# Sun-Sir/BSARec

Measured on AMD Instinct MI355X. Metric: train sequences/sec, ML-1M L=50 d=64 2-layer, higher is better.
Workload: dtype f32

## Files before the change

### bsarec_amd/csrc/fused_layer.h

```cpp
#pragma once
#include "common.h"
#include "kernels.h"
#include "wimage.h"
#include <type_traits>

#define FS 68
#define FU 260
#define FUSED_MAX_CB 8

struct FusedFwdP {
    const float* X; float* Xout;
    const float *sqrt_beta, *f_g, *f_b, *wq, *bq, *wk, *bk, *wv, *bv, *wo, *bo, *a_g, *a_b, *w1, *b1, *w2, *b2, *ff_g, *ff_b;
    const float* tw; const int* ids32;
    float *xhat_f, *rstd_f, *q, *k, *v, *probs, *ctx, *xhat_a, *rstd_a, *hmix, *u, *xhat_ff, *rstd_ff, *dsp;
    float* gp;
    int L, Lp, cb, heads;
    float alpha, oma, eps;
    DropP drop_f, drop_p, drop_o, drop_ff;
    float* trash;
    long long* stamps;
    const float *e_E, *e_pos, *e_g, *e_b; const int64_t* e_ids; GatherP e_gp; DropP e_drop; int e_V;
    float *e_X0, *e_xhat, *e_rstd; int* e_ids32;
    int xout_f32;
    const float* filter_cw;
// ... 175 lines not shown
#pragma unroll
        for (int s = 0; s < K / 16; ++s) { f.w[2 * s] = gld4(base + e + 16 * s); f.w[2 * s + 1] = gld4(base + e + 16 * s + 4); }
    } else {
#pragma unroll
        for (int kb = 0; kb < K / 8; ++kb) f.w[kb] = gld4(base + e + 8 * kb);
    }
}
template <int MM, int K, int LDW, int NR = 64, bool IMG = false>
__device__ __forceinline__ void load_wT(const float* __restrict__ base, long e, WFrag<MM, K>& f) {
    static_assert(!IMG || MM == 0, "the fragment image exists for the fp32 products only");
    if constexpr (IMG) {
        const float* gw = base + wimage_off((int)(e % LDW), (int)(e / LDW), NR);
#pragma unroll
        for (int kb = 0; kb < K / 8; ++kb) f.w[kb] = gld4(gw + 256 * kb);
    } else if constexpr (MM == 1) {
        const AS_GLOBAL unsigned short* g = reinterpret_cast<const AS_GLOBAL unsigned short*>((const AS_GLOBAL char*)base + 2 * e);
#pragma unroll
        for (int s = 0; s < K / 16; ++s) {
            unsigned h[8];
#pragma unroll
            for (int j = 0; j < 8; ++j) h[j] = g[(16 * s + j) * LDW];
            f.w[s] = u32x4{h[0] | (h[1] << 16), h[2] | (h[3] << 16), h[4] | (h[5] << 16), h[6] | (h[7] << 16)};
        }
    } else if constexpr (MM == 2) {
        const float* gw = base + e;
#pragma unroll
        for (int s = 0; s < K / 16; ++s) {
            f.w[2 * s] = f32x4{gld(gw + (16 * s + 0) * LDW), gld(gw + (16 * s + 1) * LDW), gld(gw + (16 * s + 2) * LDW), gld(gw + (16 * s + 3) * LDW)};
            f.w[2 * s + 1] = f32x4{gld(gw + (16 * s + 4) * LDW), gld(gw + (16 * s + 5) * LDW), gld(gw + (16 * s + 6) * LDW), gld(gw + (16 * s + 7) * LDW)};
        }
    } else {
        const float* gw = base + e;
#pragma unroll
        for (int kb = 0; kb < K / 8; ++kb) {
            f.w[kb].x = gld(gw + (8 * kb + 0) * LDW); f.w[kb].y = gld(gw + (8 * kb + 1) * LDW);
            f.w[kb].z = gld(gw + (8 * kb + 2) * LDW); f.w[kb].w = gld(gw + (8 * kb + 3) * LDW);
        }
    }
}
template <int MM, int K>
__device__ __forceinline__ void mma_w(const float* __restrict__ sa, const WFrag<MM, K>& f, f32x16& acc) {
    if constexpr (MM == 1) {
#pragma unroll
        for (int s = 0; s < K / 16; ++s) acc = mfma_bf16(pk8(ld4(sa + 16 * s), ld4(sa + 16 * s + 4)), f.w[s], acc);
    } else if constexpr (MM == 2) {
#pragma unroll
        for (int s = 0; s < K / 16; ++s)
            acc = mfma_x3(split3(ld4(sa + 16 * s), ld4(sa + 16 * s + 4)), split3(f.w[2 * s], f.w[2 * s + 1]), acc);
    } else {
#pragma unroll
        for (int kb = 0; kb < K / 8; ++kb) {
            const f32x4 a = ld4(sa + 8 * kb);
#pragma unroll
            for (int s = 0; s < 4; ++s) acc = __builtin_amdgcn_mfma_f32_32x32x2f32(a[s], f.w[kb][s], acc, 0, 0, 0);
        }
    }
}
template <int MM, int K>
__device__ __forceinline__ void mma_ll(const float* __restrict__ sa, const float* __restrict__ sb, f32x16& acc) {
    if constexpr (MM == 1) {
#pragma unroll
        for (int s = 0; s < K / 16; ++s)
            acc = mfma_bf16(pk8(ld4(sa + 16 * s), ld4(sa + 16 * s + 4)), pk8(ld4(sb + 16 * s), ld4(sb + 16 * s + 4)), acc);
    } else if constexpr (MM == 2) {
#pragma unroll
        for (int s = 0; s < K / 16; ++s)
            acc = mfma_x3(split3(ld4(sa + 16 * s), ld4(sa + 16 * s + 4)), split3(ld4(sb + 16 * s), ld4(sb + 16 * s + 4)), acc);
    } else {
#pragma unroll
        for (int kb = 0; kb < K / 8; ++kb) {
            const f32x4 a = ld4(sa + 8 * kb), b = ld4(sb + 8 * kb);
#pragma unroll
            for (int s = 0; s < 4; ++s) acc = __builtin_amdgcn_mfma_f32_32x32x2f32(a[s], b[s], acc, 0, 0, 0);
        }
    }
}

struct LnPre { f32x4 bi, g, be, dm[2]; };
__device__ __forceinline__ LnPre ln_pre(const float* __restrict__ bias, const float* __restrict__ gamma, const float* __restrict__ beta,
                                        const DropP& drop, const DropSeed& dseed, long tok0) {
    const int lr = threadIdx.x >> 4, lc = (threadIdx.x & 15) << 2;
    LnPre P;
    P.bi = gld4(bias + lc); P.g = gld4(gamma + lc); P.be = gld4(beta + lc);
#pragma unroll
    for (int i = 0; i < 2; ++i) P.dm[i] = drop_mult4(drop, dseed, (uint64_t)((tok0 + lr + 32 * i) * 64 + lc) >> 2);
    return P;
}
template <bool MIX, bool BF>
__device__ __forceinline__ void ln_rows_64(const LnPre& P, const float* __restrict__ tileA, const float* __restrict__ tileB,
                                           const float* __restrict__ resid, float eps, const float* __restrict__ dsp,
                                           float alpha, float oma, long tok0, int L, float* __restrict__ outL,
                                           float* __restrict__ outG, float* __restrict__ xhatG, float* __restrict__ rstdG,
                                           bool out_f32 = false ,
                                           bool round_outL = false ) {
    const int lr = threadIdx.x >> 4, lc = (threadIdx.x & 15) << 2;
#pragma unroll
    for (int i = 0; i < 2; ++i) {
        const int r = lr + 32 * i;
        const bool ok = r < L;
        const long e = (tok0 + r) * 64 + lc;
        f32x4 v = {0, 0, 0, 0};
        if (ok) v = (ld4(tileA + r * FS + lc) + ld4(tileB + r * FS + lc) + P.bi) * P.dm[i] + ld4(resid + r * FS + lc);
        const float mean = group_sum<16>(v.x + v.y + v.z + v.w) * (1.0f / 64.0f);
        f32x4 dl = {0, 0, 0, 0};
        if (ok) dl = v - mean;
        const float var = group_sum<16>(dl.x * dl.x + dl.y * dl.y + dl.z * dl.z + dl.w * dl.w) * (1.0f / 64.0f);
        const float rs = 1.0f / sqrtf(var + eps);
        f32x4 y = {0, 0, 0, 0};
        if (ok) {
            const f32x4 xh = dl * rs;
            y = P.g * xh + P.be;
            if (MIX) y = alpha * ld4(dsp + r * FS + lc) + oma * y;
            ast4<BF>(xhatG, e, xh);
            if (BF && out_f32) gst4(outG + e, y); else ast4<BF>(outG, e, y);
            if (lc == 0) gst(rstdG + tok0 + r, rs);
        }
        if (BF && round_outL) {
            const unsigned a = pk_bf16(y.x, y.y), c = pk_bf16(y.z, y.w);
            y = f32x4{bf_lo(a), bf_hi(a), bf_lo(c), bf_hi(c)};
        }
        if (outL) st4(outL + r * FS + lc, y);
    }
}

struct NoTail {};
template <bool BF> struct TopFwdRegs;
template <bool BF, unsigned KOFF, bool KV> __device__ __forceinline__ void top_fwd_prefetch(TopFwdRegs<BF>& R);
template <int DH, bool BF, unsigned KOFF, bool HELPED>
__device__ __forceinline__ void top_fwd_rest(const TopFwdRegs<BF>& R, const DropSeed& dseed, float* sX, float* sK, float* sV,
                                             float* sPart, float* sTab, float* sSpec, float* sVec, const int* sIds);
template <bool BF> struct TopFwdHelpRegs;
template <bool BF, unsigned KOFF, bool IMG> __device__ __forceinline__ void top_fwd_help_prefetch(TopFwdHelpRegs<BF>& H);
template <int DH, bool BF, unsigned KOFF>
__device__ __forceinline__ void top_fwd_help(const TopFwdHelpRegs<BF>& H, const float* sX, float* sK, float* sV, float* sVec);
template <class T> struct IsTail { static constexpr bool value = true; };
template <> struct IsTail<NoTail> { static constexpr bool value = false; };
constexpr int TOP_BWD_BARRIERS = 11;
struct TopBwdRegs {
    float sl[32];
    float xh_ff, g_ff, rs_ff, xa, xf, g_a, g_f, rs_a, rs_f, bt, low_l, x_l, q_l;
    f32x4 tq[16];
    float p_pre;
};
struct TopBwdHelpRegs { f32x4 w2c[16], w1c[16], u4; };
template <bool BF, unsigned KOFF> __device__ __forceinline__ void top_bwd_prefetch(TopBwdRegs& R);
template <bool BF, unsigned KOFF> __device__ __forceinline__ void top_bwd_prefetch_tile(TopBwdRegs& R);
template <bool BF, unsigned KOFF> __device__ __forceinline__ void top_bwd_help_prefetch(TopBwdHelpRegs& H);
template <int DH, bool BF, unsigned KOFF, bool HELPED>
__device__ __forceinline__ void top_bwd_body(const TopBwdRegs& R, const DropSeed& dseed, float* sX, float* sK, float* sV, const float* sTab,
                                             float* sVec, float* sDX);
template <bool BF, unsigned KOFF> __device__ __forceinline__ void top_bwd_help_a(const TopBwdHelpRegs& H, float* sVec);
template <int DH, bool BF, unsigned KOFF> __device__ __forceinline__ void top_bwd_help_b(const float* sX, float* sVec, const float* gu, f32x4 (&uw)[16]);


template <int DH, bool BF, class TAILP, bool X3 = false, bool FM = false, bool IMG = false>
__global__ void __launch_bounds__(512) __attribute__((amdgpu_waves_per_eu(2, 2)))
fused_layer_fwd_kernel(const FusedFwdP P_unused, const TAILP T_unused) {
#define PTYPE FusedFwdP
    static_assert(!(BF && X3), "x3 products work on fp32 tensors");
    static_assert(!IMG || (!BF && !X3 && !FM), "the fragment image feeds the fp32 products of the BSARec block");
    constexpr int MM = X3 ? 2 : (BF ? 1 : 0);
    static_assert(!FM || (!BF && !X3 && !IsTail<TAILP>::value), "the FMLPRec block runs in fp32, without a top-block tail");
    constexpr int MAXCB = FM ? 36 : FUSED_MAX_CB;
    constexpr bool TAIL = IsTail<TAILP>::value;
    constexpr unsigned KOFF = (unsigned)((sizeof(FusedFwdP) + 7) & ~(size_t)7);
    const auto R0_L = KARG(FusedFwdP, L);
    const auto R0_Lp = KARG(FusedFwdP, Lp);
    const auto R0_cb = KARG(FusedFwdP, cb);
    const auto R0_heads = KARG(FusedFwdP, heads);
    extern __shared__ __attribute__((aligned(16))) float sm[];
    constexpr int TS = 64 * FS;
    float* sX = sm;
    float* sD = sm + TS;
    float* sH = sm + 2 * TS;
    float* sE = sm + 3 * TS;
    float* sR = sm + 4 * TS;
    float* sQ = sR;
    float* sK = sR + TS;
    float* sVt = sR + 2 * TS;
    float* sC = sR + 3 * TS;
    float* sU = sR;
    float* sTab = sR + 4 * TS;
    float* sSpec = sTab + FUSED_MAX_CB * 128;
    float* sRed = sSpec + FUSED_MAX_CB * 128;
    int* sIds = reinterpret_cast<int*>(sRed + 512);
    if constexpr (FM) { sTab = sR; sSpec = sR + 2 * TS; }

    const int tid = threadIdx.x, lane = tid & 63, wave = tid >> 6;
    const int l31 = lane & 31, half = lane >> 5;
    const int grp = wave >> 2, wm = (wave >> 1) & 1, wn = wave & 1;
    const int L = R0_L, Lp = R0_Lp, heads = R0_heads, cb = R0_cb;
    const int b = blockIdx.x;
    const long tok0 = (long)b * L;
    const int col = wn * 32 + l31;
    constexpr int KHM = MM ? 8 : 4;
    const int KH = KHM * half;
    const long wrow = (long)col * 64 + KH;
    const int arow = (wm * 32 + l31) * FS + KH;
    float* const trash = KARG(FusedFwdP, trash) + 4 * lane;

    STAMP(0);
    const KernargTouch ktouch = kernarg_touch<IsTail<TAILP>::value ? KOFF + (unsigned)sizeof(TAILP) : (unsigned)sizeof(FusedFwdP)>();
    const DropSeed dseed = drop_seed(KARG(FusedFwdP, drop_f));
    kernarg_touch_done(ktouch);
    const auto R1_X = KARG(FusedFwdP, X);
    const auto R1_ids32 = KARG(FusedFwdP, ids32);
    const auto R1_tw = KARG(FusedFwdP, tw);
    const auto R1_wq = KARG(FusedFwdP, wq);
    WFrag<MM, 64> wA, wB;
    float qkv_bias[3] = {0.f, 0.f, 0.f};
    if (!FM && grp == 1) {
        load_w<MM, 64, 64, IMG>(R1_wq, wrow, wA);
        qkv_bias[0] = gld(KARG(FusedFwdP, bq) + col); qkv_bias[1] = gld(KARG(FusedFwdP, bk) + col);
        qkv_bias[2] = gld(KARG(FusedFwdP, bv) + col);
    }
    const float* const eE = KARG(FusedFwdP, e_E);
    if (eE) {
        const GatherP gp = KARG(FusedFwdP, e_gp);
        const int64_t* const eids = KARG(FusedFwdP, e_ids);
        const float* const epos = KARG(FusedFwdP, e_pos);
        const int V = KARG(FusedFwdP, e_V);
        const float eeps = KARG(FusedFwdP, eps);
        const float* const e_g = KARG(FusedFwdP, e_g); const float* const e_b = KARG(FusedFwdP, e_b);
        int* const e_ids32 = KARG(FusedFwdP, e_ids32); const DropP e_drop = KARG(FusedFwdP, e_drop);
        float* const e_xhat = KARG(FusedFwdP, e_xhat); float* const e_X0 = KARG(FusedFwdP, e_X0); float* const e_rstd = KARG(FusedFwdP, e_rstd);
        long src = 0;
        if (gp.table) {
            src = *(const AS_GLOBAL long long*)gp.cursor + b;
            src = src < gp.n ? (long)*(const AS_GLOBAL int64_t*)(gp.perm + src) : 0;
            if (tid == 0) *(AS_GLOBAL int64_t*)(gp.ans_out + b) = *(const AS_GLOBAL int64_t*)(gp.ans_table + src);
        }
        const f32x4 eg = gld4(e_g + ((tid & 15) << 2)), eb = gld4(e_b + ((tid & 15) << 2));
#pragma unroll
        for (int p = 0; p < 2; ++p) {
            const int idx = tid + p * 512, r = idx >> 4, c4 = (idx & 15) << 2;
            const bool ok = r < L;
            const long e = (tok0 + r) * 64 + c4;
            f32x4 v = {0, 0, 0, 0};
            int id = 0;
            if (ok) {
                int64_t id64;
                if (gp.table) {
                    id64 = *(const AS_GLOBAL int64_t*)(gp.table + src * L + r);
                    if (c4 == 0) *(AS_GLOBAL int64_t*)(gp.ids_out + tok0 + r) = id64;
                } else id64 = *(const AS_GLOBAL int64_t*)(eids + tok0 + r);
                id = (int)id64;
                id = id < 0 ? 0 : (id >= V ? V - 1 : id);
                v = gld4(eE + (long)id * 64 + c4) + gld4(epos + (long)r * 64 + c4);
            }
            if (c4 == 0) { sIds[r] = id; if (ok) *(AS_GLOBAL int*)(e_ids32 + tok0 + r) = id; }
            const float mean = group_sum<16>(v.x + v.y + v.z + v.w) * (1.0f / 64.0f);
            f32x4 dl = {0, 0, 0, 0};
            if (ok) dl = v - mean;
            const float var = group_sum<16>(dl.x * dl.x + dl.y * dl.y + dl.z * dl.z + dl.w * dl.w) * (1.0f / 64.0f);
            const float rs = 1.0f / sqrtf(var + eeps);
            f32x4 y = {0, 0, 0, 0};
            if (ok) {
                const f32x4 xh = dl * rs;
                y = (eg * xh + eb) * drop_mult4(e_drop, dseed, (uint64_t)e >> 2);
                ast4<BF>(e_xhat, e, xh);
                ast4<BF>(e_X0, e, y);
                if (c4 == 0) gst(e_rstd + tok0 + r, rs);
            }
            st4(sX + r * FS + c4, y);
        }
    } else {
#pragma unroll
    for (int p = 0; p < 2; ++p) {
        const int idx = tid + p * 512, r = idx >> 4, c4 = (idx & 15) << 2;
        f32x4 v = ald4<BF>(R1_X, (tok0 + min(r, L - 1)) * 64 + c4);
        if (r >= L) v = f32x4{0, 0, 0, 0};
        st4(sX + r * FS + c4, v);
    }
    if (tid < 64) sIds[tid] = tid < L ? gldi(R1_ids32 + (tok0 + tid)) : 0;
    }
    build_twiddle_table(R1_tw, L, cb, sTab);
    lds_barrier();

    STAMP(1);
    const auto R2_bk = KARG(FusedFwdP, bk);
    const auto R2_bq = KARG(FusedFwdP, bq);
    const auto R2_bv = KARG(FusedFwdP, bv);
    const auto R2_drop_f = KARG(FusedFwdP, drop_f);
    const auto R2_dsp = KARG(FusedFwdP, dsp);
    const auto R2_eps = KARG(FusedFwdP, eps);
    const auto R2_f_b = KARG(FusedFwdP, f_b);
    const auto R2_f_g = KARG(FusedFwdP, f_g);
    const auto R2_k = KARG(FusedFwdP, k);
    const auto R2_q = KARG(FusedFwdP, q);
    const auto R2_rstd_f = KARG(FusedFwdP, rstd_f);
    const auto R2_sqrt_beta = KARG(FusedFwdP, sqrt_beta);
    const auto R2_v = KARG(FusedFwdP, v);
    const auto R2_wk = KARG(FusedFwdP, wk);
    const auto R2_wo = KARG(FusedFwdP, wo);
    const auto R2_wv = KARG(FusedFwdP, wv);
    const auto R2_xhat_f = KARG(FusedFwdP, xhat_f);
    {
        float* part = sH;
        const int lr = (tid & 255) >> 4, lc = (tid & 15) << 2;
        auto qkv = [&](auto whichc) {
            constexpr int which = decltype(whichc)::value;
            f32x16 acc;
#pragma unroll
            for (int r = 0; r < 16; ++r) acc[r] = 0.f;
            if (which == 0) { load_w<MM, 64, 64, IMG>(R2_wk, wrow, wB); mma_w<MM, 64>(sX + arow, wA, acc); }
            else if (which == 1) { load_w<MM, 64, 64, IMG>(R2_wv, wrow, wA); mma_w<MM, 64>(sX + arow, wB, acc); }
            else mma_w<MM, 64>(sX + arow, wA, acc);
            const float bias = qkv_bias[which];
#pragma unroll
            for (int r = 0; r < 16; ++r) {
                const int row = wm * 32 + rho(r) + 4 * half;
                const float val = acc[r] + bias;
                if (which == 0) sQ[row * FS + col] = val;
                else if (which == 1) sK[row * FS + col] = val;
                else sVt[col * FS + row] = val;
            }
        };
#pragma unroll
        for (int ch = 0; ch < MAXCB / 4; ++ch) {
            const int k0 = 4 * ch;
            if (k0 >= cb) break;
            if (grp == 0) {
                f32x4 re[4], im[4];
#pragma unroll
                for (int j = 0; j < 4; ++j) { re[j] = f32x4{0, 0, 0, 0}; im[j] = f32x4{0, 0, 0, 0}; }
#pragma unroll
                for (int r0 = 0; r0 < 64; r0 += 16) {
                    const int t = r0 + lr;
                    if (t < L) {
                        const f32x4 x = ld4(sX + t * FS + lc);
#pragma unroll
                        for (int j = 0; j < 4; ++j)
                            if (k0 + j < cb) {
                                const float c = sTab[2 * ((k0 + j) * 64 + t)], sn = sTab[2 * ((k0 + j) * 64 + t) + 1];
                                re[j] += x * c; im[j] -= x * sn;
                            }
                    }
                }
#pragma unroll
                for (int j = 0; j < 4; ++j) {
                    st4(part + ((lr * 4 + j) * 2 + 0) * 64 + lc, re[j]);
                    st4(part + ((lr * 4 + j) * 2 + 1) * 64 + lc, im[j]);
                }
            } else if (!FM && ch == 0) qkv(std::integral_constant<int, 0>{});
            lds_barrier();
            if (grp == 0) {
                for (int i = tid; i < 512; i += 256) {
                    const int j = i >> 7, rc = i & 127;
                    if (k0 + j < cb) {
                        float acc = 0.f;
#pragma unroll
                        for (int g = 0; g < 16; ++g) acc += part[g * 512 + i];
                        sSpec[(k0 + j) * 128 + rc] = acc;
                    }
                }
            } else if (!FM && ch == 0) qkv(std::integral_constant<int, 1>{});
            lds_barrier();
        }
        if (!FM && grp == 1) qkv(std::integral_constant<int, 2>{});
        if constexpr (FM) {
            const float* const cwp = KARG(FusedFwdP, filter_cw);
            for (int i = tid; i < cb * 64; i += 512) {
                const int k = i >> 6, c = i & 63;
                const float xr = sSpec[k * 128 + c], xi = sSpec[k * 128 + 64 + c];
                const float wr = gld(cwp + 2 * i), wi = gld(cwp + 2 * i + 1);
                sSpec[k * 128 + c] = xr * wr - xi * wi;
                sSpec[k * 128 + 64 + c] = xr * wi + xi * wr;
            }
            lds_barrier();
        }
        {
            f32x4 b2 = gld4(R2_sqrt_beta + lc);
            b2 = b2 * b2;
            if constexpr (FM) b2 = f32x4{0, 0, 0, 0};
            float* const R2_hmix = KARG(FusedFwdP, hmix);
            const f32x4 g = gld4(R2_f_g + lc), be = gld4(R2_f_b + lc);
            const int rbeg = grp == 0 ? 0 : 48, rend = grp == 0 ? 48 : 64;
            for (int r0 = rbeg; r0 < rend; r0 += 16) {
                const int t = r0 + lr;
                const bool ok = t < L;
                const long e = (tok0 + t) * 64 + lc;
                f32x4 v = {0, 0, 0, 0};
                if (ok) {
                    const f32x4 xv = ld4(sX + t * FS + lc);
                    const f32x4 low = lowpass_tab(sSpec, t, lc, L, cb, sTab);
                    v = (low + b2 * (xv - low)) * drop_mult4(R2_drop_f, dseed, (uint64_t)e >> 2) + xv;
                }
                const float mean = group_sum<16>(v.x + v.y + v.z + v.w) * (1.0f / 64.0f);
                f32x4 dl = {0, 0, 0, 0};
                if (ok) dl = v - mean;
                const float var = group_sum<16>(dl.x * dl.x + dl.y * dl.y + dl.z * dl.z + dl.w * dl.w) * (1.0f / 64.0f);
                const float rs = 1.0f / sqrtf(var + R2_eps);
                f32x4 y = {0, 0, 0, 0};
                if (ok) {
                    const f32x4 xh = dl * rs;
                    y = g * xh + be;
                    ast4<BF>(R2_xhat_f, e, xh);
                    if (R2_dsp) gst4(R2_dsp + e, y);
                    if constexpr (FM) gst4(R2_hmix + e, y);
                    if (lc == 0) gst(R2_rstd_f + (tok0 + t), rs);
                }
                st4((FM ? sH : sD) + t * FS + lc, y);
            }
        }
    }
    WFrag<MM, 32> wO;
    if constexpr (!FM) load_w<MM, 32, 64, IMG>(R2_wo, wrow + 32 * grp, wO);
    lds_barrier();
    if constexpr (!FM) {
    {
        const int lr = tid >> 4, lc = (tid & 15) << 2;
#pragma unroll
        for (int r0 = 0; r0 < 64; r0 += 32) {
            const int r = r0 + lr;
            if (r < L) {
                const long e = (tok0 + r) * 64 + lc;
                ast4<BF>(R2_q, e, ld4(sQ + r * FS + lc));
                ast4<BF>(R2_k, e, ld4(sK + r * FS + lc));
                ast4<BF>(R2_v, e, f32x4{sVt[lc * FS + r], sVt[(lc + 1) * FS + r], sVt[(lc + 2) * FS + r], sVt[(lc + 3) * FS + r]});
            }
        }
    }

    STAMP(3);
    const auto R3_ctx = KARG(FusedFwdP, ctx);
    const auto R3_drop_p = KARG(FusedFwdP, drop_p);
    const auto R3_probs = KARG(FusedFwdP, probs);
    {
        const int nt = (L + 31) >> 5;
        const float sqrt_dh = sqrtf((float)DH);
        constexpr int NCT = (DH + 31) / 32;
        const int ncombo = heads * nt;
        const int pair = wave >> 1, kt = wave & 1;
        for (int c0 = 0; c0 < ncombo; c0 += 4) {
            const int combo = c0 + pair;
            const bool act = combo < ncombo && kt < nt;
            const int head = act ? combo / nt : 0, qt = act ? combo % nt : 0;
            const int query = 32 * qt + l31;
            f32x16 st;
#pragma unroll
            for (int r = 0; r < 16; ++r) st[r] = 0.f;
            float mx = -INFINITY;
            if (act) {
                mma_ll<MM, DH>(sK + (32 * kt + l31) * FS + head * DH + KH, sQ + query * FS + head * DH + KH, st);
#pragma unroll
                for (int r = 0; r < 16; ++r) {
                    const int key = 32 * kt + rho(r) + 4 * half;
                    float s = -INFINITY;
                    if (key < L) s = st[r] / sqrt_dh + ((key <= query && sIds[key] > 0) ? 0.0f : -10000.0f);
                    st[r] = s;
                    mx = fmaxf(mx, s);
                }
                mx = xor32_max(mx);
                sRed[(pair * 2 + kt) * 64 + lane] = mx;
            }
            lds_barrier();
            float sum = 0.f;
            if (act) {
                if (nt == 2) mx = fmaxf(mx, sRed[(pair * 2 + (kt ^ 1)) * 64 + lane]);
#pragma unroll
                for (int r = 0; r < 16; ++r) {
                    const int key = 32 * kt + rho(r) + 4 * half;
                    const float e = key < L ? __expf(st[r] - mx) : 0.f;
                    st[r] = e;
                    sum += e;
                }
                sum = xor32_sum(sum);
            }
            lds_barrier();
            if (act) sRed[(pair * 2 + kt) * 64 + lane] = sum;
            lds_barrier();
            if (act) {
                if (nt == 2) sum += sRed[(pair * 2 + (kt ^ 1)) * 64 + lane];
                const float inv = 1.0f / sum;
#pragma unroll
                for (int g = 0; g < 4; ++g) {
                    const int key0 = 32 * kt + 8 * g + 4 * half;
                    f32x4 p = {st[4 * g] * inv, st[4 * g + 1] * inv, st[4 * g + 2] * inv, st[4 * g + 3] * inv};
                    f32x4 m = {1.f, 1.f, 1.f, 1.f};
                    if (query < L && key0 < Lp) {
                        const long e = (((long)b * heads + head) * L + query) * Lp + key0;
                        ast4<BF>(R3_probs, e, p);
                        m = drop_mult4(R3_drop_p, dseed, (uint64_t)e >> 2);
                    }
                    p = p * m;
                    st[4 * g] = p.x; st[4 * g + 1] = p.y; st[4 * g + 2] = p.z; st[4 * g + 3] = p.w;
                }
                float* dstT = kt == 0 ? sC : sE;
#pragma unroll
                for (int ct = 0; ct < NCT; ++ct) {
                    f32x16 cacc;
#pragma unroll
                    for (int r = 0; r < 16; ++r) cacc[r] = 0.f;
                    const bool crow_ok = 32 * ct + l31 < DH;
                    const float* va = sVt + (head * DH + 32 * ct + (crow_ok ? l31 : 0)) * FS + 32 * kt + 4 * half;
                    if constexpr (MM != 0) {
#pragma unroll
                        for (int s2 = 0; s2 < 2; ++s2) {
                            f32x4 a0 = ld4(va + 16 * s2), a1 = ld4(va + 16 * s2 + 8);
                            if (!crow_ok) { a0 = f32x4{0, 0, 0, 0}; a1 = a0; }
                            if constexpr (MM == 1) {
                                const u32x4 pb = {pk_bf16(st[8 * s2], st[8 * s2 + 1]), pk_bf16(st[8 * s2 + 2], st[8 * s2 + 3]),
                                                  pk_bf16(st[8 * s2 + 4], st[8 * s2 + 5]), pk_bf16(st[8 * s2 + 6], st[8 * s2 + 7])};
                                cacc = mfma_bf16(pk8(a0, a1), pb, cacc);
                            } else {
                                cacc = mfma_x3(split3(a0, a1), split3(f32x4{st[8 * s2], st[8 * s2 + 1], st[8 * s2 + 2], st[8 * s2 + 3]},
                                                                      f32x4{st[8 * s2 + 4], st[8 * s2 + 5], st[8 * s2 + 6], st[8 * s2 + 7]}), cacc);
                            }
                        }
                    } else {
#pragma unroll
                    for (int g = 0; g < 4; ++g) {
                        f32x4 a = ld4(va + 8 * g);
                        if (!crow_ok) a = f32x4{0, 0, 0, 0};
#pragma unroll
                        for (int j = 0; j < 4; ++j)
                            cacc = __builtin_amdgcn_mfma_f32_32x32x2f32(a[j], st[4 * g + j], cacc, 0, 0, 0);
                    }
                    }
#pragma unroll
                    for (int g = 0; g < 4; ++g) {
                        const int c = 32 * ct + 8 * g + 4 * half;
                        if (c < DH)
                            st4(dstT + query * FS + head * DH + c, f32x4{cacc[4 * g], cacc[4 * g + 1], cacc[4 * g + 2], cacc[4 * g + 3]});
                    }
                }
            }
            lds_barrier();
        }
        {
            const int lr = tid >> 4, lc = (tid & 15) << 2;
#pragma unroll
            for (int r0 = 0; r0 < 64; r0 += 32) {
                const int r = r0 + lr;
                f32x4 v = {0, 0, 0, 0};
                if (r < 32 * nt) { v = ld4(sC + r * FS + lc); if (nt == 2) v += ld4(sE + r * FS + lc); }
                st4(sC + r * FS + lc, v);
                if (r < L) ast4<BF>(R3_ctx, (tok0 + r) * 64 + lc, v);
            }
        }
    }
    lds_barrier();
    }

    STAMP(4);
    const auto R4_a_b = KARG(FusedFwdP, a_b);
    const auto R4_a_g = KARG(FusedFwdP, a_g);
    const auto R4_alpha = KARG(FusedFwdP, alpha);
    const auto R4_bo = KARG(FusedFwdP, bo);
    const auto R4_drop_o = KARG(FusedFwdP, drop_o);
    const auto R4_eps = KARG(FusedFwdP, eps);
    const auto R4_hmix = KARG(FusedFwdP, hmix);
    const auto R4_oma = KARG(FusedFwdP, oma);
    const auto R4_rstd_a = KARG(FusedFwdP, rstd_a);
    const auto R4_w1 = KARG(FusedFwdP, w1);
    const auto R4_xhat_a = KARG(FusedFwdP, xhat_a);
    float ffn_bias[2];
    LnPre lnA;
    if constexpr (!FM) lnA = ln_pre(R4_bo, R4_a_g, R4_a_b, R4_drop_o, dseed, tok0);
    {
        load_w<MM, 64, 64, IMG>(R4_w1, (long)(128 * grp + col) * 64 + KH, wA);
        ffn_bias[0] = gld(KARG(FusedFwdP, b1) + 128 * grp + col); ffn_bias[1] = gld(KARG(FusedFwdP, b1) + 128 * grp + 64 + col);
        if constexpr (!FM) {
        f32x16 acc;
#pragma unroll
        for (int r = 0; r < 16; ++r) acc[r] = 0.f;
        mma_w<MM, 32>(sC + arow + 32 * grp, wO, acc);
        float* part = grp == 0 ? sQ : sK;
#pragma unroll
        for (int r = 0; r < 16; ++r) part[(wm * 32 + rho(r) + 4 * half) * FS + col] = acc[r];
        }
    }
    if constexpr (!FM) {
    lds_barrier();
    ln_rows_64<true, BF>(lnA, sQ, sK, sX, R4_eps, sD, R4_alpha, R4_oma, tok0, L, sH, R4_hmix, R4_xhat_a, R4_rstd_a);
    lds_barrier();
    }

    STAMP(5);
    const auto R5_b1 = KARG(FusedFwdP, b1);
    const auto R5_u = KARG(FusedFwdP, u);
    const auto R5_w1 = KARG(FusedFwdP, w1);
    const auto R5_w2 = KARG(FusedFwdP, w2);
    {
        const float* sa = sH + arow;
#pragma unroll
        for (int i = 0; i < 2; ++i) {
            const int c256 = (2 * grp + i) * 64 + col;
            WFrag<MM, 64>& wcur = i ? wB : wA;
            WFrag<MM, 64>& wnxt = i ? wA : wB;
            if (i == 0) load_w<MM, 64, 64, IMG>(R5_w1, (long)(c256 + 64) * 64 + KH, wnxt);
            else load_w<MM, 64, 256, IMG>(R5_w2, (long)col * 256 + 128 * grp + KH, wnxt);
            f32x16 acc;
#pragma unroll
            for (int r = 0; r < 16; ++r) acc[r] = 0.f;
            mma_w<MM, 64>(sa, wcur, acc);
            const float bias = ffn_bias[i];
#pragma unroll
            for (int r = 0; r < 16; ++r) {
                const int row = wm * 32 + rho(r) + 4 * half;
                sU[row * FU + c256] = acc[r] + bias;
            }
        }
    }
    lds_barrier();

    STAMP(6);
    const auto R6_w2 = KARG(FusedFwdP, w2);
    const auto R6_u = KARG(FusedFwdP, u);
    const auto R6_gp = KARG(FusedFwdP, gp);
    const auto R7_b2 = KARG(FusedFwdP, b2);
    const auto R7_drop_ff = KARG(FusedFwdP, drop_ff);
    const auto R7_ff_b = KARG(FusedFwdP, ff_b);
    const auto R7_ff_g = KARG(FusedFwdP, ff_g);
    LnPre lnF;
    {
        for (int idx = tid; idx < 64 * 64; idx += 512) {
            const int r = idx >> 6, c4 = (idx & 63) << 2;
            const f32x4 v = ld4(sU + r * FU + c4);
            float g0, g1, g2, g3, p0, p1, p2, p3;
            gelu_both(v.x, g0, p0); gelu_both(v.y, g1, p1); gelu_both(v.z, g2, p2); gelu_both(v.w, g3, p3);
            const f32x4 g = {g0, g1, g2, g3}, gp = {p0, p1, p2, p3};
            if (r < L) { ast4<BF>(R6_u, (tok0 + r) * 256 + c4, g); ast4<BF>(R6_gp, (tok0 + r) * 256 + c4, gp); }
            st4(sU + r * FU + c4, g);
        }
        lds_barrier();
        lnF = ln_pre(R7_b2, R7_ff_g, R7_ff_b, R7_drop_ff, dseed, tok0);
        f32x16 acc;
#pragma unroll
        for (int r = 0; r < 16; ++r) acc[r] = 0.f;
        const float* sa = sU + (wm * 32 + l31) * FU + 128 * grp + KH;
        load_w<MM, 64, 256, IMG>(R6_w2, (long)col * 256 + 128 * grp + 64 + KH, wB);
        mma_w<MM, 64>(sa, wA, acc);
        mma_w<MM, 64>(sa + 64, wB, acc);
        float* part = grp == 0 ? sX : sE;
#pragma unroll
        for (int r = 0; r < 16; ++r) part[(wm * 32 + rho(r) + 4 * half) * FS + col] = acc[r];
    }
    lds_barrier();
    STAMP(7);
    TopFwdRegs<BF> TR;
    TopFwdHelpRegs<BF> TH;
    if constexpr (TAIL) { if (wave < 4) top_fwd_prefetch<BF, KOFF, false>(TR); else top_fwd_help_prefetch<BF, KOFF, IMG>(TH); }
    const auto R7_Xout = KARG(FusedFwdP, Xout);
    const auto R7_eps = KARG(FusedFwdP, eps);
    const auto R7_rstd_ff = KARG(FusedFwdP, rstd_ff);
    const auto R7_xhat_ff = KARG(FusedFwdP, xhat_ff);
    ln_rows_64<false, BF>(lnF, sX, sE, sH, R7_eps, nullptr, 0.f, 1.f, tok0, L,
                          TAIL ? sD : nullptr, R7_Xout, R7_xhat_ff, R7_rstd_ff, KARG(FusedFwdP, xout_f32) != 0, TAIL);
    STAMP(8);
    if constexpr (TAIL) {
        lds_barrier();
        if (wave < 4) top_fwd_rest<DH, BF, KOFF, true>(TR, dseed, sD, sR, sR + TS, sR + 2 * TS, sTab, sSpec, sX, sIds);
        else top_fwd_help<DH, BF, KOFF>(TH, sD, sR, sR + TS, sX);
    }
}
#undef PTYPE

static inline size_t fused_fwd_smem_bytes() {
    return (size_t)(8 * 64 * FS + 2 * FUSED_MAX_CB * 128 + 512 + 64) * 4;
}

struct FusedBwdP {
    const float* dY; float* dX; const float* X;
    const float *sqrt_beta, *f_g, *wq, *wk, *wv, *wo, *a_g, *w1, *w2, *ff_g;
    const float* tw;
    const float *xhat_f, *rstd_f, *q, *k, *v, *probs, *xhat_a, *rstd_a, *u, *xhat_ff, *rstd_ff;
    const float* dh_slabs; int dh_nsplit; long dh_stride;
    float *dT, *dU, *dO, *dq, *dk, *dv;
    float *pg_ff, *pb_ff, *pg_a, *pb_a, *pg_f, *pb_f, *pbeta;
    int L, Lp, cb, heads;
    float alpha, oma;
    DropP drop_f, drop_p, drop_o, drop_ff;
    float* trash;
    long long* stamps;
    float* e_dz; const float *e_xhat, *e_rstd, *e_g; float *e_pg, *e_pb; DropP e_drop;
    const float* filter_cw; float* pcw;
    const float* e_dx_extra;
};


__device__ __forceinline__ void seq_partial_64(const f32x4& v, float* __restrict__ red, float* __restrict__ dst, float scale_by = 1.f,
                                               const float* __restrict__ mul = nullptr) {
    const int lr = threadIdx.x >> 4, lc = (threadIdx.x & 15) << 2;
    const int ng = blockDim.x >> 4;
    lds_barrier();
    st4(red + lr * 64 + lc, v);
    lds_barrier();
    if (threadIdx.x < 64) {
        float s = 0.f;
        for (int g = 0; g < ng; ++g) s += red[g * 64 + threadIdx.x];
        if (mul) s *= gld(mul + threadIdx.x);
        gst(dst + threadIdx.x, s * scale_by);
    }
}


template <int N>
__device__ __forceinline__ void seq_partials_64(const f32x4 (&v)[N], float* const (&red)[N], float* const (&dst)[N],
                                                float scale0 = 1.f, const float* __restrict__ mul0 = nullptr) {
    const int lr = threadIdx.x >> 4, lc = (threadIdx.x & 15) << 2;
    const int ng = blockDim.x >> 4;
    lds_barrier();
#pragma unroll
    for (int i = 0; i < N; ++i) st4(red[i] + lr * 64 + lc, v[i]);
    lds_barrier();
    const int i = threadIdx.x >> 6, c = threadIdx.x & 63;
    if (i < N) {
        const float* r = red[0];
        float* d = dst[0];
#pragma unroll
        for (int k = 1; k < N; ++k) if (i == k) { r = red[k]; d = dst[k]; }
        float s0 = 0.f, s1 = 0.f, s2 = 0.f, s3 = 0.f;
        for (int g = 0; g < ng; g += 4) {
            s0 += r[g * 64 + c]; s1 += r[(g + 1) * 64 + c]; s2 += r[(g + 2) * 64 + c]; s3 += r[(g + 3) * 64 + c];
        }
        float sum = (s0 + s1) + (s2 + s3);
        if (i == 0) { if (mul0) sum *= gld(mul0 + c); sum *= scale0; }
        gst(d + c, sum);
    }
}

template <int DH, bool BF, class HEADP, bool X3 = false, bool FM = false, bool IMG = false>
__global__ void __launch_bounds__(512) __attribute__((amdgpu_waves_per_eu(2, 2)))
fused_layer_bwd_kernel(const FusedBwdP P_unused, const HEADP H_unused) {
#define PTYPE FusedBwdP
    static_assert(!(BF && X3), "x3 products work on fp32 tensors");
    static_assert(!IMG || (!BF && !X3 && !FM), "the fragment image feeds the fp32 products of the BSARec block");
    constexpr int MM = X3 ? 2 : (BF ? 1 : 0);
    static_assert(!FM || (!BF && !X3 && !IsTail<HEADP>::value), "the FMLPRec block runs in fp32, without a top-block head");
    constexpr bool HEAD = IsTail<HEADP>::value;
    constexpr unsigned KOFF = (unsigned)((sizeof(FusedBwdP) + 7) & ~(size_t)7);
    const auto R0_L = KARG(FusedBwdP, L);
    const auto R0_Lp = KARG(FusedBwdP, Lp);
    const auto R0_cb = KARG(FusedBwdP, cb);
    const auto R0_heads = KARG(FusedBwdP, heads);
    extern __shared__ __attribute__((aligned(16))) float sm[];
    constexpr int TS = 64 * FS;
    float* sAcc = sm;
    float* sT = sm + TS;
    float* sQ = sm + 2 * TS;
    float* sK = sm + 3 * TS;
    float* sV = sm + 4 * TS;
    float* sS = sm + 5 * TS;
    float* sdU = sQ;
    float* sG = sm + 6 * TS;
    float* sdF = sm + 7 * TS;
    float* sPm = sm + 8 * TS;
    float* sTab = sm + 9 * TS;
    float* sRed = sTab + FUSED_MAX_CB * 128;
    const int tid = threadIdx.x, lane = tid & 63, wave = tid >> 6;
    const int l31 = lane & 31, half = lane >> 5;
    const int grp = wave >> 2, wm = (wave >> 1) & 1, wn = wave & 1;
    const int lr = tid >> 4, lc = (tid & 15) << 2;
    const int L = R0_L, Lp = R0_Lp, heads = R0_heads, cb = R0_cb;
    const int b = blockIdx.x;
    const long tok0 = (long)b * L;
    const int col = wn * 32 + l31;
    constexpr int KHM = MM ? 8 : 4;
    const int KH = KHM * half;
    const int arow = (wm * 32 + l31) * FS + KH;
    float* const trash = KARG(FusedBwdP, trash) + 4 * lane;

    STAMP(0);
    const KernargTouch ktouch = kernarg_touch<KOFF + (unsigned)sizeof(HEADP)>();
    TopBwdRegs HR;
    TopBwdHelpRegs HH;
    if constexpr (HEAD) {
        if (wave == 0) top_bwd_prefetch<BF, KOFF>(HR);
        else if (wave < 4) {
            if (wave == 3) build_twiddle_table(KARG(FusedBwdP, tw), L, cb, sTab, 192, 64);
            top_bwd_prefetch_tile<BF, KOFF>(HR);
        } else top_bwd_help_prefetch<BF, KOFF>(HH);
    }
    const DropSeed dseed = drop_seed(KARG(FusedBwdP, drop_f));
    kernarg_touch_done(ktouch);
    const auto R1_dT = KARG(FusedBwdP, dT);
    const auto R1_dY = KARG(FusedBwdP, dY);
    const auto R1_dh_nsplit = KARG(FusedBwdP, dh_nsplit);
    const auto R1_dh_slabs = KARG(FusedBwdP, dh_slabs);
    const auto R1_dh_stride = KARG(FusedBwdP, dh_stride);
    const auto R1_drop_ff = KARG(FusedBwdP, drop_ff);
    const auto R1_ff_g = KARG(FusedBwdP, ff_g);
    const auto R1_pb_ff = KARG(FusedBwdP, pb_ff);
    const auto R1_pg_ff = KARG(FusedBwdP, pg_ff);
    const auto R1_rstd_ff = KARG(FusedBwdP, rstd_ff);
    const auto R1_tw = KARG(FusedBwdP, tw);
    const auto R1_w2 = KARG(FusedBwdP, w2);
    const auto R1_xhat_ff = KARG(FusedBwdP, xhat_ff);
    if constexpr (!FM && !HEAD) build_twiddle_table(R1_tw, L, cb, sTab);
    if constexpr (HEAD) {
        if (wave < 4) {
            top_bwd_body<DH, BF, KOFF, true>(HR, dseed, sG, sdF, sPm, sTab, sAcc, sT);
        } else {
            top_bwd_help_a<BF, KOFF>(HH, sAcc);
            f32x4 uw[16];
            top_bwd_help_b<DH, BF, KOFF>(sG, sAcc, KARG(FusedBwdP, u), uw);
#pragma unroll
            for (int i = 0; i < 16; ++i) {
                const int idx = (tid - 256) + i * 256, r = idx >> 6, c4 = (idx & 63) << 2;
                st4(sdU + r * FU + c4, r < L ? uw[i] : f32x4{0, 0, 0, 0});
            }
        }
    }
    WFrag<MM, 64> wA, wB;
    WFrag<MM, 32> wk4;
    f32x4 e_bt, e_x[2];
    load_wT<MM, 64, 256, 64, IMG>(R1_w2, (long)KH * 256 + 128 * grp + col, wA);
    const f32x4 g = gld4(R1_ff_g + lc);
    f32x4 dy[2], xh[2];
    float rs[2];
#pragma unroll
    for (int i = 0; i < 2; ++i) {
        const int r = 32 * i + lr;
        const long e = (tok0 + r) * 64 + lc;
        dy[i] = f32x4{0, 0, 0, 0}; xh[i] = dy[i]; rs[i] = 0.f;
        if (R1_dh_slabs) {
            if (r < L) {
                if (r == L - 1)
                    for (int sp = 0; sp < R1_dh_nsplit; ++sp) dy[i] += gld4(R1_dh_slabs + sp * R1_dh_stride + (long)b * 64 + lc);
                xh[i] = ald4<BF>(R1_xhat_ff, e); rs[i] = gld(R1_rstd_ff + tok0 + r);
            }
        } else {
            const bool ok = r < L;
            const long ec = (tok0 + min(r, L - 1)) * 64 + lc;
            f32x4 d4 = {0, 0, 0, 0};
            if constexpr (!HEAD) d4 = ald4<BF>(R1_dY, ec);
            const f32x4 x4 = ald4<BF>(R1_xhat_ff, ec);
            const float r1 = gld(R1_rstd_ff + tok0 + min(r, L - 1));
            if constexpr (HEAD) d4 = ld4(sT + r * FS + lc);
            dy[i] = ok ? d4 : f32x4{0, 0, 0, 0}; xh[i] = ok ? x4 : f32x4{0, 0, 0, 0}; rs[i] = ok ? r1 : 0.f;
        }
    }
    f32x4 uv[8];
    if constexpr (!HEAD)
    {
        const float* gu = KARG(FusedBwdP, u);
#pragma unroll
        for (int i = 0; i < 8; ++i) {
            const int idx = tid + i * 512, r = idx >> 6, c4 = (idx & 63) << 2;
            uv[i] = ald4<BF>(gu, (tok0 + min(r, L - 1)) * 256 + c4);
        }
    }

    {
        f32x4 sg = {0, 0, 0, 0}, sb = sg;
#pragma unroll
        for (int i = 0; i < 2; ++i) {
            const int r = 32 * i + lr;
            const bool ok = r < L;
            const long e = (tok0 + r) * 64 + lc;
            const f32x4 gg = dy[i] * g;
            const float m1 = group_sum<16>(gg.x + gg.y + gg.z + gg.w) * (1.0f / 64.0f);
            const float m2 = group_sum<16>(gg.x * xh[i].x + gg.y * xh[i].y + gg.z * xh[i].z + gg.w * xh[i].w) * (1.0f / 64.0f);
            const f32x4 dz = rs[i] * (gg - m1 - xh[i] * m2);
            sg += dy[i] * xh[i]; sb += dy[i];
            f32x4 dt = {0, 0, 0, 0};
            if (ok) { dt = dz * drop_mult4(R1_drop_ff, dseed, (uint64_t)e >> 2); ast4<BF>(R1_dT, e, dt); }
            st4(sAcc + r * FS + lc, dz);
            st4(sT + r * FS + lc, dt);
        }
        {
            const f32x4 pv[2] = {sg, sb};
            float* const pr[2] = {sPm, sPm + 2048};
            float* const pd[2] = {R1_pg_ff + (long)b * 64, R1_pb_ff + (long)b * 64};
            seq_partials_64<2>(pv, pr, pd);
        }
    }
    if constexpr (!HEAD) {
#pragma unroll
    for (int i = 0; i < 8; ++i) {
        const int idx = tid + i * 512, r = idx >> 6, c4 = (idx & 63) << 2;
        st4(sdU + r * FU + c4, r < L ? uv[i] : f32x4{0, 0, 0, 0});
// ... 608 lines not shown
```

Before: 1.726 million.

## Use 16-row MFMA attention tiles without cross-wave reductions in fp32 forward

```diff
diff --git a/bsarec_amd/csrc/fused_layer.h b/bsarec_amd/csrc/fused_layer.h
--- a/bsarec_amd/csrc/fused_layer.h
+++ b/bsarec_amd/csrc/fused_layer.h
@@ -351,6 +351,90 @@
 template <bool BF, unsigned KOFF> __device__ __forceinline__ void top_bwd_help_a(const TopBwdHelpRegs& H, float* sVec);
 template <int DH, bool BF, unsigned KOFF> __device__ __forceinline__ void top_bwd_help_b(const float* sX, float* sVec, const float* gu, f32x4 (&uw)[16]);
 
+
+template <int DH, int NK, bool BF>
+__device__ __forceinline__ void attend_16(const float* sQ, const float* sK, const float* sVt, float* sC, const int* sIds, int L, int Lp,
+                                          int heads, int b, float* __restrict__ probs, uint32_t drop_thresh, float drop_scale,
+                                          uint32_t drop_site, const DropSeed& dseed) {
+    const DropP drop_p = {drop_thresh, drop_scale, nullptr, drop_site};
+    const int lane = threadIdx.x & 63, wave = threadIdx.x >> 6;
+    const int n = lane & 15, g4 = (lane >> 4) << 2;
+    const float sqrt_dh = sqrtf((float)DH);
+    constexpr int NF = DH / 16;
+    for (int combo = wave; combo < heads * NK; combo += 8) {
+        const int head = combo / NK, hc = head * DH;
+        const int query = 16 * (combo % NK) + n;
+        f32x4 qf[NF], st[NK];
+#pragma unroll
+        for (int f = 0; f < NF; ++f) qf[f] = ld4(sQ + query * FS + hc + 16 * f + g4);
+#pragma unroll
+        for (int t = 0; t < NK; ++t) st[t] = f32x4{0, 0, 0, 0};
+        const float* const ka = sK + n * FS + hc + g4;
+#pragma unroll
+        for (int f = 0; f < NF; ++f) {
+            f32x4 a[NK];
+#pragma unroll
+            for (int t = 0; t < NK; ++t) a[t] = ld4(ka + 16 * t * FS + 16 * f);
+#pragma unroll
+            for (int j = 0; j < 4; ++j)
+#pragma unroll
+                for (int t = 0; t < NK; ++t)
+                    st[t] = __builtin_amdgcn_mfma_f32_16x16x4f32(a[t][j], qf[f][j], st[t], 0, 0, 0);
+        }
+        float mx = -INFINITY;
+#pragma unroll
+        for (int t = 0; t < NK; ++t)
+#pragma unroll
+            for (int i = 0; i < 4; ++i) {
+                const int key = 16 * t + g4 + i;
+                float s = -INFINITY;
+                if (key < L) s = st[t][i] / sqrt_dh + ((key <= query && sIds[key] > 0) ? 0.0f : -10000.0f);
+                st[t][i] = s;
+                mx = fmaxf(mx, s);
+            }
+        mx = quad_rows_max(mx);
+        float sum = 0.f;
+#pragma unroll
+        for (int t = 0; t < NK; ++t)
+#pragma unroll
+            for (int i = 0; i < 4; ++i) {
+                const float e = 16 * t + g4 + i < L ? __expf(st[t][i] - mx) : 0.f;
+                st[t][i] = e;
+                sum += e;
+            }
+        sum = quad_rows_sum(sum);
+        const float inv = 1.0f / sum;
+#pragma unroll
+        for (int t = 0; t < NK; ++t) {
+            const int key0 = 16 * t + g4;
+            f32x4 p = st[t] * inv;
+            f32x4 m = {1.f, 1.f, 1.f, 1.f};
+            if (query < L && key0 < Lp) {
+                const long e = (((long)b * heads + head) * L + query) * Lp + key0;
+                ast4<BF>(probs, e, p);
+                m = drop_mult4(drop_p, dseed, (uint64_t)e >> 2);
+            }
+            st[t] = p * m;
+        }
+        f32x4 cacc[NF];
+#pragma unroll
+        for (int f = 0; f < NF; ++f) cacc[f] = f32x4{0, 0, 0, 0};
+        const float* const va = sVt + (hc + n) * FS + g4;
+#pragma unroll
+        for (int t = 0; t < NK; ++t) {
+            f32x4 a[NF];
+#pragma unroll
+            for (int f = 0; f < NF; ++f) a[f] = ld4(va + 16 * f * FS + 16 * t);
+#pragma unroll
+            for (int j = 0; j < 4; ++j)
+#pragma unroll
+                for (int f = 0; f < NF; ++f)
+                    cacc[f] = __builtin_amdgcn_mfma_f32_16x16x4f32(a[f][j], st[t][j], cacc[f], 0, 0, 0);
+        }
+#pragma unroll
+        for (int f = 0; f < NF; ++f) st4(sC + query * FS + hc + 16 * f + g4, cacc[f]);
+    }
+}
 
 template <int DH, bool BF, class TAILP, bool X3 = false, bool FM = false, bool IMG = false>
 __global__ void __launch_bounds__(512) __attribute__((amdgpu_waves_per_eu(2, 2)))
@@ -626,74 +710,94 @@
     const auto R3_drop_p = KARG(FusedFwdP, drop_p);
     const auto R3_probs = KARG(FusedFwdP, probs);
     {
-        const int nt = (L + 31) >> 5;
-        const float sqrt_dh = sqrtf((float)DH);
-        constexpr int NCT = (DH + 31) / 32;
-        const int ncombo = heads * nt;
-        const int pair = wave >> 1, kt = wave & 1;
-        for (int c0 = 0; c0 < ncombo; c0 += 4) {
-            const int combo = c0 + pair;
-            const bool act = combo < ncombo && kt < nt;
-            const int head = act ? combo / nt : 0, qt = act ? combo % nt : 0;
-            const int query = 32 * qt + l31;
-            f32x16 st;
-#pragma unroll
-            for (int r = 0; r < 16; ++r) st[r] = 0.f;
-            float mx = -INFINITY;
-            if (act) {
-                mma_ll<MM, DH>(sK + (32 * kt + l31) * FS + head * DH + KH, sQ + query * FS + head * DH + KH, st);
-#pragma unroll
-                for (int r = 0; r < 16; ++r) {
-                    const int key = 32 * kt + rho(r) + 4 * half;
-                    float s = -INFINITY;
-                    if (key < L) s = st[r] / sqrt_dh + ((key <= query && sIds[key] > 0) ? 0.0f : -10000.0f);
-                    st[r] = s;
-                    mx = fmaxf(mx, s);
-                }
-                mx = xor32_max(mx);
-                sRed[(pair * 2 + kt) * 64 + lane] = mx;
-            }
-            lds_barrier();
-            float sum = 0.f;
-            if (act) {
-                if (nt == 2) mx = fmaxf(mx, sRed[(pair * 2 + (kt ^ 1)) * 64 + lane]);
-#pragma unroll
-                for (int r = 0; r < 16; ++r) {
-                    const int key = 32 * kt + rho(r) + 4 * half;
-                    const float e = key < L ? __expf(st[r] - mx) : 0.f;
-                    st[r] = e;
-                    sum += e;
-                }
-                sum = xor32_sum(sum);
-            }
-            lds_barrier();
-            if (act) sRed[(pair * 2 + kt) * 64 + lane] = sum;
-            lds_barrier();
-            if (act) {
-                if (nt == 2) sum += sRed[(pair * 2 + (kt ^ 1)) * 64 + lane];
-                const float inv = 1.0f / sum;
-#pragma unroll
-                for (int g = 0; g < 4; ++g) {
-                    const int key0 = 32 * kt + 8 * g + 4 * half;
-                    f32x4 p = {st[4 * g] * inv, st[4 * g + 1] * inv, st[4 * g + 2] * inv, st[4 * g + 3] * inv};
-                    f32x4 m = {1.f, 1.f, 1.f, 1.f};
-                    if (query < L && key0 < Lp) {
-                        const long e = (((long)b * heads + head) * L + query) * Lp + key0;
-                        ast4<BF>(R3_probs, e, p);
-                        m = drop_mult4(R3_drop_p, dseed, (uint64_t)e >> 2);
+        if constexpr (MM == 0) {
+        const int nq = (L + 15) >> 4;
+        switch (nq) {
+            case 1: attend_16<DH, 1, BF>(sQ, sK, sVt, sC, sIds, L, Lp, heads, b, R3_probs, R3_drop_p.thresh, R3_drop_p.scale, R3_drop_p.site, dseed); break;
+            case 2: attend_16<DH, 2, BF>(sQ, sK, sVt, sC, sIds, L, Lp, heads, b, R3_probs, R3_drop_p.thresh, R3_drop_p.scale, R3_drop_p.site, dseed); break;
+            case 3: attend_16<DH, 3, BF>(sQ, sK, sVt, sC, sIds, L, Lp, heads, b, R3_probs, R3_drop_p.thresh, R3_drop_p.scale, R3_drop_p.site, dseed); break;
+            default: attend_16<DH, 4, BF>(sQ, sK, sVt, sC, sIds, L, Lp, heads, b, R3_probs, R3_drop_p.thresh, R3_drop_p.scale, R3_drop_p.site, dseed); break;
+        }
+        lds_barrier();
+        {
+            const int lr = tid >> 4, lc = (tid & 15) << 2;
+#pragma unroll
+            for (int r0 = 0; r0 < 64; r0 += 32) {
+                const int r = r0 + lr;
+                f32x4 v = {0, 0, 0, 0};
+                if (r < 16 * nq) v = ld4(sC + r * FS + lc);
+                else st4(sC + r * FS + lc, v);
+                if (r < L) ast4<BF>(R3_ctx, (tok0 + r) * 64 + lc, v);
+            }
+        }
+        } else {
+            const int nt = (L + 31) >> 5;
+            const float sqrt_dh = sqrtf((float)DH);
+            constexpr int NCT = (DH + 31) / 32;
+            const int ncombo = heads * nt;
+            const int pair = wave >> 1, kt = wave & 1;
+            for (int c0 = 0; c0 < ncombo; c0 += 4) {
+                const int combo = c0 + pair;
+                const bool act = combo < ncombo && kt < nt;
+                const int head = act ? combo / nt : 0, qt = act ? combo % nt : 0;
+                const int query = 32 * qt + l31;
+                f32x16 st;
+#pragma unroll
+                for (int r = 0; r < 16; ++r) st[r] = 0.f;
+                float mx = -INFINITY;
+                if (act) {
+                    mma_ll<MM, DH>(sK + (32 * kt + l31) * FS + head * DH + KH, sQ + query * FS + head * DH + KH, st);
+#pragma unroll
+                    for (int r = 0; r < 16; ++r) {
+                        const int key = 32 * kt + rho(r) + 4 * half;
+                        float s = -INFINITY;
+                        if (key < L) s = st[r] / sqrt_dh + ((key <= query && sIds[key] > 0) ? 0.0f : -10000.0f);
+                        st[r] = s;
+                        mx = fmaxf(mx, s);
                     }
-                    p = p * m;
-                    st[4 * g] = p.x; st[4 * g + 1] = p.y; st[4 * g + 2] = p.z; st[4 * g + 3] = p.w;
-                }
-                float* dstT = kt == 0 ? sC : sE;
-#pragma unroll
-                for (int ct = 0; ct < NCT; ++ct) {
-                    f32x16 cacc;
-#pragma unroll
-                    for (int r = 0; r < 16; ++r) cacc[r] = 0.f;
-                    const bool crow_ok = 32 * ct + l31 < DH;
-                    const float* va = sVt + (head * DH + 32 * ct + (crow_ok ? l31 : 0)) * FS + 32 * kt + 4 * half;
-                    if constexpr (MM != 0) {
+                    mx = xor32_max(mx);
+                    sRed[(pair * 2 + kt) * 64 + lane] = mx;
+                }
+                lds_barrier();
+                float sum = 0.f;
+                if (act) {
+                    if (nt == 2) mx = fmaxf(mx, sRed[(pair * 2 + (kt ^ 1)) * 64 + lane]);
+#pragma unroll
+                    for (int r = 0; r < 16; ++r) {
+                        const int key = 32 * kt + rho(r) + 4 * half;
+                        const float e = key < L ? __expf(st[r] - mx) : 0.f;
+                        st[r] = e;
+                        sum += e;
+                    }
+                    sum = xor32_sum(sum);
+                }
+                lds_barrier();
+                if (act) sRed[(pair * 2 + kt) * 64 + lane] = sum;
+                lds_barrier();
+                if (act) {
+                    if (nt == 2) sum += sRed[(pair * 2 + (kt ^ 1)) * 64 + lane];
+                    const float inv = 1.0f / sum;
+#pragma unroll
+                    for (int g = 0; g < 4; ++g) {
+                        const int key0 = 32 * kt + 8 * g + 4 * half;
+                        f32x4 p = {st[4 * g] * inv, st[4 * g + 1] * inv, st[4 * g + 2] * inv, st[4 * g + 3] * inv};
+                        f32x4 m = {1.f, 1.f, 1.f, 1.f};
+                        if (query < L && key0 < Lp) {
+                            const long e = (((long)b * heads + head) * L + query) * Lp + key0;
+                            ast4<BF>(R3_probs, e, p);
+                            m = drop_mult4(R3_drop_p, dseed, (uint64_t)e >> 2);
+                        }
+                        p = p * m;
+                        st[4 * g] = p.x; st[4 * g + 1] = p.y; st[4 * g + 2] = p.z; st[4 * g + 3] = p.w;
+                    }
+                    float* dstT = kt == 0 ? sC : sE;
+#pragma unroll
+                    for (int ct = 0; ct < NCT; ++ct) {
+                        f32x16 cacc;
+#pragma unroll
+                        for (int r = 0; r < 16; ++r) cacc[r] = 0.f;
+                        const bool crow_ok = 32 * ct + l31 < DH;
+                        const float* va = sVt + (head * DH + 32 * ct + (crow_ok ? l31 : 0)) * FS + 32 * kt + 4 * half;
 #pragma unroll
                         for (int s2 = 0; s2 < 2; ++s2) {
                             f32x4 a0 = ld4(va + 16 * s2), a1 = ld4(va + 16 * s2 + 8);
@@ -707,35 +811,26 @@
                                                                       f32x4{st[8 * s2 + 4], st[8 * s2 + 5], st[8 * s2 + 6], st[8 * s2 + 7]}), cacc);
                             }
                         }
-                    } else {
-#pragma unroll
-                    for (int g = 0; g < 4; ++g) {
-                        f32x4 a = ld4(va + 8 * g);
-                        if (!crow_ok) a = f32x4{0, 0, 0, 0};
-#pragma unroll
-                        for (int j = 0; j < 4; ++j)
-                            cacc = __builtin_amdgcn_mfma_f32_32x32x2f32(a[j], st[4 * g + j], cacc, 0, 0, 0);
+#pragma unroll
+                        for (int g = 0; g < 4; ++g) {
+                            const int c = 32 * ct + 8 * g + 4 * half;
+                            if (c < DH)
+                                st4(dstT + query * FS + head * DH + c, f32x4{cacc[4 * g], cacc[4 * g + 1], cacc[4 * g + 2], cacc[4 * g + 3]});
+                        }
                     }
-                    }
-#pragma unroll
-                    for (int g = 0; g < 4; ++g) {
-                        const int c = 32 * ct + 8 * g + 4 * half;
-                        if (c < DH)
-                            st4(dstT + query * FS + head * DH + c, f32x4{cacc[4 * g], cacc[4 * g + 1], cacc[4 * g + 2], cacc[4 * g + 3]});
-                    }
-                }
-            }
-            lds_barrier();
-        }
-        {
-            const int lr = tid >> 4, lc = (tid & 15) << 2;
-#pragma unroll
-            for (int r0 = 0; r0 < 64; r0 += 32) {
-                const int r = r0 + lr;
-                f32x4 v = {0, 0, 0, 0};
-                if (r < 32 * nt) { v = ld4(sC + r * FS + lc); if (nt == 2) v += ld4(sE + r * FS + lc); }
-                st4(sC + r * FS + lc, v);
-                if (r < L) ast4<BF>(R3_ctx, (tok0 + r) * 64 + lc, v);
+                }
+                lds_barrier();
+            }
+            {
+                const int lr = tid >> 4, lc = (tid & 15) << 2;
+#pragma unroll
+                for (int r0 = 0; r0 < 64; r0 += 32) {
+                    const int r = r0 + lr;
+                    f32x4 v = {0, 0, 0, 0};
+                    if (r < 32 * nt) { v = ld4(sC + r * FS + lc); if (nt == 2) v += ld4(sE + r * FS + lc); }
+                    st4(sC + r * FS + lc, v);
+                    if (r < L) ast4<BF>(R3_ctx, (tok0 + r) * 64 + lc, v);
+                }
             }
         }
     }
@@ -814,13 +909,13 @@
     const auto R7_ff_g = KARG(FusedFwdP, ff_g);
     LnPre lnF;
     {
-        for (int idx = tid; idx < 64 * 64; idx += 512) {
+        for (int idx = tid; idx < L * 64; idx += 512) {
             const int r = idx >> 6, c4 = (idx & 63) << 2;
             const f32x4 v = ld4(sU + r * FU + c4);
             float g0, g1, g2, g3, p0, p1, p2, p3;
             gelu_both(v.x, g0, p0); gelu_both(v.y, g1, p1); gelu_both(v.z, g2, p2); gelu_both(v.w, g3, p3);
             const f32x4 g = {g0, g1, g2, g3}, gp = {p0, p1, p2, p3};
-            if (r < L) { ast4<BF>(R6_u, (tok0 + r) * 256 + c4, g); ast4<BF>(R6_gp, (tok0 + r) * 256 + c4, gp); }
+            ast4<BF>(R6_u, (tok0 + r) * 256 + c4, g); ast4<BF>(R6_gp, (tok0 + r) * 256 + c4, gp);
             st4(sU + r * FU + c4, g);
         }
         lds_barrier();
@@ -904,20 +999,19 @@
 #pragma unroll
     for (int i = 0; i < N; ++i) st4(red[i] + lr * 64 + lc, v[i]);
     lds_barrier();
-    const int i = threadIdx.x >> 6, c = threadIdx.x & 63;
-    if (i < N) {
-        const float* r = red[0];
-        float* d = dst[0];
-#pragma unroll
-        for (int k = 1; k < N; ++k) if (i == k) { r = red[k]; d = dst[k]; }
-        float s0 = 0.f, s1 = 0.f, s2 = 0.f, s3 = 0.f;
-        for (int g = 0; g < ng; g += 4) {
-            s0 += r[g * 64 + c]; s1 += r[(g + 1) * 64 + c]; s2 += r[(g + 2) * 64 + c]; s3 += r[(g + 3) * 64 + c];
-        }
-        float sum = (s0 + s1) + (s2 + s3);
-        if (i == 0) { if (mul0) sum *= gld(mul0 + c); sum *= scale0; }
-        gst(d + c, sum);
-    }
+    const int i = __builtin_amdgcn_readfirstlane(threadIdx.x >> 6), c = threadIdx.x & 63;
+#pragma unroll
+    for (int k = 0; k < N; ++k)
+        if (i == k) {
+            const float* const r = red[k];
+            float s0 = 0.f, s1 = 0.f, s2 = 0.f, s3 = 0.f;
+            for (int g = 0; g < ng; g += 4) {
+                s0 += r[g * 64 + c]; s1 += r[(g + 1) * 64 + c]; s2 += r[(g + 2) * 64 + c]; s3 += r[(g + 3) * 64 + c];
+            }
+            float sum = (s0 + s1) + (s2 + s3);
+            if (k == 0) { if (mul0) sum *= gld(mul0 + c); sum *= scale0; }
+            gst(dst[k] + c, sum);
+        }
 }
 
 template <int DH, bool BF, class HEADP, bool X3 = false, bool FM = false, bool IMG = false>
```

Result: no change. 1.733 million (median of 6 runs) (+0.4%).
